# tszalay/poreseq

Hardware: AMD Instinct MI355X
Metric: kb consensus refined/sec at 10x coverage (higher is better)
Workload: dtype f64; 1 GPU; poreseq consensus, 10 kb region, 10x synthetic coverage (BASELINE configs[1]), full Mutate.py schedule per region; a step is 280 independent regions per GPU = 14 lock-step batches; the batches of the timed steps run step by step (a step's batches all finish before the next step's start) through 14 batch slots (host threads) per GPU; marshalling + H2D of the events, host greedy steps and D2H inside; region_bases=10000, events=10, regions_per_gpu=280, batches_in_flight=14, step_barrier=True, parallelism=280 regions x 1 GPU(s), 14 host thread(s) per GPU, no data-path collective

## Files before the change

poreseq_amd/csrc/ps_find.cpp:

```cpp
#include <algorithm>
#include <cmath>
#include <cstdlib>
#include <cstring>
#include <map>
#include <thread>

#include "ps_extract.h"
#include "ps_host.h"
#include "ps_sw.h"

namespace ps {

static bool likes_on_host() { const char* e = getenv("PORESEQ_DEBUG_LIKES_HOST"); return e && atoi(e) != 0; }

static void fillinds(SwResult& al) {
    if (al.a.empty()) return;
    int i1 = al.a[0], i2 = al.b[0];
    for (size_t k = 0; k < al.a.size(); k++) {
        if (al.a[k] > 0) i1 = al.a[k]; else al.a[k] = i1;
        if (al.b[k] > 0) i2 = al.b[k]; else al.b[k] = i2;
    }
}

namespace {
// ... 214 lines not shown
    for (size_t i = 1; i < st.size(); i++) {
        if (cur == st[i]) continue;
        bool hit = false;
        for (int n = 1; n <= 4 && !hit; n++)
            for (int k = 0; k < (1 << (2 * n)); k++)
                if (succ(cur, k, n) == st[i]) {
                    for (int b = 1; b <= n; b++) s.push_back(base_at(cur, b));
                    cur = st[i]; hit = true; break;
                }
        if (!hit) { cur = st[i]; s.push_back(base_at(cur, 0)); }
    }
    for (int b = 1; b <= 4; b++) s.push_back(base_at(cur, b));
    return s;
}

struct RandState {
    random_data rd;
    char st[128];
    bool init = false;
};
namespace { thread_local RandState t_rand; }
static void rs_seed(RandState* r, unsigned seed) {
    memset(&r->rd, 0, sizeof(r->rd));
    initstate_r(seed, r->st, sizeof(r->st), &r->rd);
    r->init = true;
}
static int rs_next(RandState* r) {
    if (!r->init) rs_seed(r, 1);
    int32_t v = 0;
    random_r(&r->rd, &v);
    return (int)v;
}
void rand_seed(unsigned seed) { rs_seed(&t_rand, seed); }
int rand_next() { return rs_next(&t_rand); }
RandState* rand_state_new(unsigned seed) { RandState* r = new RandState(); rs_seed(r, seed); return r; }
void rand_state_free(RandState* r) { delete r; }
void rand_state_seed(RandState* r, unsigned seed) { rs_seed(r, seed); }
int rand_state_next(RandState* r) { return rs_next(r ? r : &t_rand); }

namespace {
struct VitGather { std::vector<double> obsin; int T = 0; };
}

static int vit_refuses_refs(const Align& a, const char* who, int region) {
    for (int e = 0; e < a.E; e++) {
        const double* ra = a.h_ra.data() + a.off[e];
        for (int t = 0; t < a.n[e]; t++)
            if (ra[t] >= 2147483648.0) {
                char val[64];
                snprintf(val, sizeof(val), "%g", ra[t]);
                return fail(PS_ERR_BAD_ARG, std::string(who) + ": " + (region >= 0 ? "region " + std::to_string(region) + ": " : std::string()) + "event " + std::to_string(e) +
                                                ", level " + std::to_string(t) + ": ref_align = " + val + " is not below 2^31 (ViterbiMutate walks the positions from (int)ref_align)");
            }
    }
    return PS_OK;
}

static void vit_gather(const Align* a, const double* h_ri, const JobOut* info, VitGather* g) {
    const int E = a->E;
    int maxpos = 0;
    for (int e = 0; e < E; e++) {
        if (!info[e].has_index) continue;
        const double* ri = h_ri + a->off[e];
        for (int t = 0; t < a->n[e]; t++) {
            const double v = ri[t];
            if (v >= 0.0 && v < 1e9 && v == std::floor(v)) maxpos = std::max(maxpos, (int)v);
        }
    }
    std::vector<std::vector<int>> first(E);
    for (int e = 0; e < E; e++) {
        if (!info[e].has_index) continue;
        first[e].assign((size_t)maxpos + 2, -1);
        const double* ri = h_ri + a->off[e];
        for (int t = 0; t < a->n[e]; t++) {
            const double v = ri[t];
            if (v >= -1.0 && v <= (double)maxpos && v == std::floor(v)) {
                int& slot = first[e][(size_t)((int)v + 1)];
                if (slot < 0) slot = t;
            }
        }
    }
    auto rstart = [&](int e) { return info[e].has_index ? info[e].refstart : -1; };
    auto rend = [&](int e) { return info[e].has_index ? info[e].refend : -1; };
    int refind = rstart(0);
    for (int e = 0; e < E; e++) refind = std::min(refind, rstart(e));
    std::vector<double>& obsin = g->obsin;
    int T = 0;
    while (true) {
        int nl = 0, nal = 0;
        const size_t at = obsin.size();
        obsin.resize(at + (size_t)E * 4, 0.0);
        for (int e = 0; e < E; e++) {
            if (refind < -1 || refind > maxpos || first[e].empty() || first[e][refind + 1] < 0) continue;
            const double* ra = a->h_ra.data() + a->off[e];
            const double* mean = a->h_mean.data() + a->off[e];
            const double* stdv = a->h_stdv.data() + a->off[e];
            int t = first[e][refind + 1], cnt = 1;
            double lsum = 0, ssum = 0;
            lsum += mean[t]; ssum += stdv[t];
            for (t++; t < a->n[e] && ra[t] <= refind; t++)
                if (ra[t] > 0) { lsum += mean[t]; ssum += stdv[t]; cnt++; }
            const double lvl = lsum / cnt, sd = ssum / cnt;
            nl++;
            double* o = obsin.data() + at + (size_t)e * 4;
            o[0] = lvl; o[1] = sd; o[2] = std::log(sd); o[3] = 1.0;
        }
        for (int e = 0; e < E; e++) if (refind >= rstart(e) && refind <= rend(e)) nal++;
        if (nl <= nal * 0.2) {
            obsin.resize(at);
            if (nal == 0) break;
            refind++;
            continue;
        }
        T++;
        refind++;
    }
    g->T = T;
}

static void vit_draw(void* rng, double* rnd, size_t n) {
    RandState* r = (RandState*)rng;
    for (size_t k = 0; k < n; k++) rnd[k] = rand_state_next(r) / (double(RAND_MAX) + 1);
}

int viterbi_mutate_multi(Runtime* rt, const std::vector<Align*>& as, const std::vector<RandState*>& rngs, int nkeep, double skip, double stay,
                         double mmin, double mmax, const std::vector<std::vector<std::string>*>& outs, VitTap* tap, const char* who, bool lockstep) {
    Tick tk("viterbi_mutate");
    const int R = (int)as.size();
    for (int r = 0; r < R; r++) outs[r]->clear();
    std::vector<double*> h_ri(R, nullptr);
    std::vector<JobOut*> info(R, nullptr);
    for (int r = 0; r < R; r++) {
        PS_TRY(as[r]->refs_to_host_async(rt));
        as[r]->last_stream = (void*)rt->stream;
        PS_TRY(rt->down(&h_ri[r], as[r]->d_ri, (size_t)as[r]->ntot));
        PS_TRY(rt->down(&info[r], as[r]->d_out, (size_t)as[r]->E));
    }
    PS_HIP(hipStreamSynchronize(rt->stream));
    for (int r = 0; r < R; r++) as[r]->refs_finish();
    tk.lap("refs D2H");
    for (int r = 0; r < R; r++) PS_TRY(vit_refuses_refs(*as[r], who, lockstep ? r : -1));
    std::vector<VitGather> gath(R);
    par_for(R, [&](int r) { vit_gather(as[r], h_ri[r], info[r], &gath[r]); });
    tk.lap("gather levels");
    std::vector<VitRegionH> regs(R);
    for (int r = 0; r < R; r++) {
        regs[r].E = as[r]->E; regs[r].T = gath[r].T; regs[r].obsin = gath[r].obsin.data(); regs[r].d_model = as[r]->d_model;
        as[r]->last_stream = (void*)rt->stream;
        regs[r].rng = rngs[r]; regs[r].draw = vit_draw;
        regs[r].index = lockstep ? r : -1;
    }
    std::vector<std::vector<std::vector<int>>> paths;
    {
        auto need = [&](size_t k) { return 26.0 * 1024.0 * (double)regs[k].T + 32.0 * (double)regs[k].T * regs[k].E; };
        double cap = std::max(1e9, PLAN_VITERBI_FRAC * device_share_bytes());
        for (size_t k0 = 0; k0 < regs.size();) {
            size_t k1 = k0;
            double acc = 0;
            for (; k1 < regs.size(); k1++) { const double add = need(k1); if (k1 > k0 && acc + add > cap) break; acc += add; }
            std::vector<std::vector<std::vector<int>>> part;
            const int rc = viterbi_device_multi(rt, std::vector<VitRegionH>(regs.begin() + k0, regs.begin() + k1), nkeep, skip, stay, mmin, mmax, &part, tap, who);
            if (rc == PS_ERR_NOMEM && k1 - k0 > 1) { cap *= 0.5; continue; }
            PS_TRY(rc);
            for (auto& pr : part) paths.push_back(std::move(pr));
            k0 = k1;
        }
    }
    tk.lap("device");
    par_for(R, [&](int r) { for (auto& p : paths[r]) outs[r]->push_back(path_to_bases(p)); });
    tk.lap("paths to bases");
    return PS_OK;
}

int viterbi_mutate(Runtime* rt, Align* a, int nkeep, double skip, double stay, double mmin, double mmax,
                   std::vector<std::string>* out, bool verbose) {
    const int rc = viterbi_mutate_multi(rt, {a}, {nullptr}, nkeep, skip, stay, mmin, mmax, {out}, nullptr, "ps_viterbi_mutate", false);
    if (verbose && rc == PS_OK) {
        fputs("Viterbi", stderr);
        for (size_t k = 200; k <= a->bases.size(); k += 200) fputc('.', stderr);
        fputc('\n', stderr);
        fflush(stderr);
    }
    return rc;
}

}
```

poreseq_amd/csrc/ps_poison.h:

```cpp
#ifndef PS_POISON_H_
#define PS_POISON_H_

#include <cstring>

namespace ps {

enum class PoisonClass { INDEX = 0, VALUE = 1, EXEMPT = 2 };
struct PoisonEntry { const char* name; PoisonClass cls; const char* why; };

constexpr PoisonEntry POISON_TABLE[] = {
    {"jobs", PoisonClass::INDEX, "JobD: pointers, sizes, offsets"},
    {"states", PoisonClass::INDEX, "5-mer state ids and their -1 padding"},
    {"lb", PoisonClass::INDEX, "band centres per column"},
    {"lo", PoisonClass::INDEX, "lowest in-band row per anti-diagonal"},
    {"hi", PoisonClass::INDEX, "highest in-band row per anti-diagonal"},
    {"maxw", PoisonClass::INDEX, "widest footprint: sizes P"},
    {"fill_pairs", PoisonClass::INDEX, "job indices of paired fills"},
    {"rec", PoisonClass::INDEX, "records {main, stay} — and the Viterbi arena, whose back-pointer shorts the host follows as state ids (vit_follow_bp)"},
    {"flg", PoisonClass::INDEX, "step words and strip codes: the backtrace turns them into moves"},
    {"cmax", PoisonClass::VALUE, "per-column maxima of main: read by k_prefix and the edit kernels as max operands only"},
    {"pm", PoisonClass::VALUE, "prefix maxima over columns: compared and added, never indexed with"},
    {"best", PoisonClass::VALUE, "JobOut.best gathered per job: copied to the host and clamped at 0"},
    {"sw_jobs", PoisonClass::INDEX, "SweepJob: offsets and step counts"},
    {"sw_band", PoisonClass::INDEX, "row bounds per column"},
    {"sw_qlo", PoisonClass::INDEX, "lowest strip in band per step"},
    {"sw_qhi", PoisonClass::INDEX, "highest strip in band per step"},
    {"sw_sb", PoisonClass::INDEX, "StripBest: score with its cell"},
    {"sw_win", PoisonClass::INDEX, "widest window of strips: sizes the launch"},
    {"sw_pairs", PoisonClass::INDEX, "SwPair: lengths and offsets"},
    {"sw_chars", PoisonClass::INDEX, "sequence bytes, compared and used as substitution keys"},
    {"sw_row", PoisonClass::INDEX, "checkpoint rows of packed scores and directions"},
    {"sw_col", PoisonClass::INDEX, "checkpoint columns"},
    {"sw_blk", PoisonClass::INDEX, "block maxima with their cells"},
    {"sw_prog", PoisonClass::INDEX, "progress counters the blocks spin on"},
    {"sw_out", PoisonClass::INDEX, "index lists"},
    {"sw_res", PoisonClass::INDEX, "per-pair records: score, cell, list length"},
    {"sw_map_redo", PoisonClass::INDEX, "position tables of redone pairs"},
    {"seed_refs", PoisonClass::INDEX, "ref_align doubles are converted to column indices"},
    {"seed_out", PoisonClass::INDEX, "JobOut: cells and flags beside the score"},
    {"like_groups", PoisonClass::INDEX, "LikeGroup: job ranges and offsets"},
    {"like_out", PoisonClass::VALUE, "per-base likelihood sums: copied to the host and differenced"},
    {"remap_units", PoisonClass::INDEX, "unit descriptors of k_remap"},
    {"var_map", PoisonClass::INDEX, "position tables"},
    {"keep", PoisonClass::INDEX, "kept-column index per column"},
    {"mutint", PoisonClass::INDEX, "edit tables and descriptors"},
    {"mutdbl", PoisonClass::VALUE, "old / delta / score / oldall doubles: max and sum operands, copied to the host as scores"},
    {"ptable", PoisonClass::INDEX, "ps_point_best carries slots beside the scores"},
    {"support", PoisonClass::INDEX, "records with counts"},
    {"phase", PoisonClass::INDEX, "links, set ids, haplotype tags"},
    {"astats_in", PoisonClass::INDEX, "StatJob / StatRegion: pointers and sizes"},
    {"astats", PoisonClass::INDEX, "ps_event_stats and ps_kmer_cell carry counts"},
    {"vit_regs", PoisonClass::INDEX, "VitReg: pointers, sizes, offsets"},
    {"vit_posreg", PoisonClass::INDEX, "region of every position"},
    {"vit_in", PoisonClass::INDEX, "the fourth double of every record is the `present` flag"},
    {"vit_lik", PoisonClass::VALUE, "final scores per state: the host takes their argmax, a comparison of values"},
    {"vit_att", PoisonClass::INDEX, "default"},
    {"vit_start", PoisonClass::INDEX, "start state of the traces"},
    {"vit_rnd", PoisonClass::INDEX, "deviates: the picked state depends on them"},
    {"vit_path", PoisonClass::INDEX, "state paths"},
};

inline const PoisonEntry* poison_entry(const char* name) {
    for (const PoisonEntry& e : POISON_TABLE) if (!strcmp(e.name, name)) return &e;
    return nullptr;
}

}

#endif
```

poreseq_amd/csrc/ps_viterbi.hip:

```cpp
#include <atomic>

#include "ps_internal.h"
#include "ps_vitpath.h"

namespace ps {

struct ModelRowV { double mu, sg, lsg, sm, lam, llam; };
__device__ __forceinline__ double emission_v(const ModelRowV& m, double x, double sd, double lsd, double log2pi) {
    double d = (x - m.mu) / m.sg;
    double l = -0.5 * (d * d + log2pi) - m.lsg;
    double e = (sd - m.sm) / m.sm;
    l += 0.5 * (m.llam - 3 * lsd - log2pi - e * e * m.lam / sd);
    return l;
}

struct VitReg {
    const double* model;
    int E, T;
    int64_t in_off;
    int64_t t_off;
};

template <int VMAXE>
__global__ __launch_bounds__(256) void k_vit_obs(const VitReg* __restrict__ regs, const int* __restrict__ pos_reg, const double* __restrict__ obsin,
                                                 double log2pi, double* __restrict__ obs, double* __restrict__ eobs) {
    const int t = blockIdx.x;
    const VitReg R = regs[pos_reg[t]];
    const int E = R.E;
    const double* in = obsin + R.in_off + (size_t)(t - R.t_off) * E * 4;
    for (int st = threadIdx.x; st < NS; st += 256) {
        double v[VMAXE];
        int nl = 0;
        for (int e = 0; e < E; e++) {
            if (in[e * 4 + 3] == 0.0) continue;
            const double* gm = R.model + (size_t)e * 6 * NS;
            ModelRowV m = {gm[st], gm[NS + st], gm[2 * NS + st], gm[3 * NS + st], gm[4 * NS + st], gm[5 * NS + st]};
            const double l = emission_v(m, in[e * 4 + 0], in[e * 4 + 1], in[e * 4 + 2], log2pi);
            int k = nl++;
            while (k > 0 && v[k - 1] > l) { v[k] = v[k - 1]; k--; }
            v[k] = l;
        }
        double r;
        if (nl > 1) {
            int drop = (int)floor(nl * 0.25);
            if (drop > nl - 2) drop = 0;
            double s = 0.0;
            for (int k = drop; k < nl; k++) s += v[k];
            r = s / (double)(nl - drop);
        } else {
            r = nl == 1 ? v[0] : 0.0;
        }
        obs[(size_t)t * NS + st] = r;
        eobs[(size_t)t * NS + st] = exp(r);
    }
}

__global__ __launch_bounds__(256) void k_vit_obs_lds(const VitReg* __restrict__ regs, const int* __restrict__ pos_reg, const double* __restrict__ obsin,
                                                     double log2pi, double* __restrict__ obs, double* __restrict__ eobs) {
    extern __shared__ double vit_v[];
    const int t = blockIdx.x;
    const VitReg R = regs[pos_reg[t]];
    const int E = R.E;
    const double* in = obsin + R.in_off + (size_t)(t - R.t_off) * E * 4;
    double* v = vit_v + threadIdx.x;
    for (int st = threadIdx.x; st < NS; st += 256) {
        int nl = 0;
        for (int e = 0; e < E; e++) {
            if (in[e * 4 + 3] == 0.0) continue;
            const double* gm = R.model + (size_t)e * 6 * NS;
            ModelRowV m = {gm[st], gm[NS + st], gm[2 * NS + st], gm[3 * NS + st], gm[4 * NS + st], gm[5 * NS + st]};
            const double l = emission_v(m, in[e * 4 + 0], in[e * 4 + 1], in[e * 4 + 2], log2pi);
            int k = nl++;
            while (k > 0) {
                const double w = v[(k - 1) * 256];
                if (!(w > l)) break;
                v[k * 256] = w;
                k--;
            }
            v[k * 256] = l;
        }
        double r;
        if (nl > 1) {
            int drop = (int)floor(nl * 0.25);
            if (drop > nl - 2) drop = 0;
            double s = 0.0;
            for (int k = drop; k < nl; k++) s += v[k * 256];
            r = s / (double)(nl - drop);
        } else {
            r = nl == 1 ? v[0] : 0.0;
        }
        obs[(size_t)t * NS + st] = r;
        eobs[(size_t)t * NS + st] = exp(r);
    }
}

#define PS_LDS_BARRIER() asm volatile("s_waitcnt lgkmcnt(0)\n\ts_barrier" ::: "memory")

struct Fam { double mx, second, psum; int idx; int pad; };

__device__ __forceinline__ Fam fam_join(const Fam& A, const Fam& B) {
    Fam r;
    r.mx = fmax(A.mx, B.mx);
    const int ia = A.mx == r.mx ? A.idx : 0x7fffffff, ib = B.mx == r.mx ? B.idx : 0x7fffffff;
    r.idx = min(ia, ib);
    const double lower = A.mx == B.mx ? -BIG * 10 : fmin(A.mx, B.mx);
    r.second = fmax(fmax(A.second, B.second), lower);
    r.psum = A.psum + B.psum;
    r.pad = 0;
    return r;
}

template <int N>
__device__ __forceinline__ double row_shl(double v) {
    int lo = __double2loint(v), hi = __double2hiint(v);
    lo = __builtin_amdgcn_update_dpp(0, lo, 0x100 + N, 0xf, 0xf, true);
    hi = __builtin_amdgcn_update_dpp(0, hi, 0x100 + N, 0xf, 0xf, true);
    return __hiloint2double(hi, lo);
}
template <int N>
__device__ __forceinline__ Fam fam_shl(const Fam& f) {
    Fam o;
    o.mx = row_shl<N>(f.mx); o.second = row_shl<N>(f.second); o.psum = row_shl<N>(f.psum);
    o.idx = __builtin_amdgcn_update_dpp(0, f.idx, 0x100 + N, 0xf, 0xf, true); o.pad = 0;
    return o;
}
__device__ __forceinline__ double wave_sum(double v) {
    v += row_shl<1>(v); v += row_shl<2>(v); v += row_shl<4>(v); v += row_shl<8>(v);
    auto lane_d = [&](int l) {
        const int lo = __builtin_amdgcn_readlane(__double2loint(v), l), hi = __builtin_amdgcn_readlane(__double2hiint(v), l);
        return __hiloint2double(hi, lo);
    };
    return (lane_d(0) + lane_d(16)) + (lane_d(32) + lane_d(48));
}

__device__ __forceinline__ double below(double x) {
    long long b = __double_as_longlong(x);
    b += x < 0.0 ? 1 : -1;
    return __longlong_as_double(b);
}

#define VPAD(q) ((q) + ((q) >> 5))

__global__ __launch_bounds__(1024) void k_vit_steps(const VitReg* __restrict__ regs, const double* __restrict__ obs_all, const double* __restrict__ eobs_all,
                                                    double skip, double stay, double lskip, double lstay, double l25,
                                                    short* __restrict__ bp_all, double* __restrict__ lfwd_all,
                                                    double* __restrict__ lik_final_all, int keep_fwd) {
    const int T = regs[blockIdx.x].T;
    const size_t roff = (size_t)regs[blockIdx.x].t_off * NS;
    const double* __restrict__ obs = obs_all + roff;
    const double* __restrict__ eobs = eobs_all + roff;
    short* __restrict__ bp = bp_all + roff;
    double* __restrict__ lfwd_out = lfwd_all + (keep_fwd ? roff : 0);
    double* __restrict__ lik_final = lik_final_all + (size_t)blockIdx.x * NS;
    if (T <= 0) return;
    __shared__ double s_lik[2][NS + NS / 32], s_fwd[2][NS + NS / 32];
    __shared__ Fam s_fam[336];
    __shared__ double s_red[16];
    __shared__ double s_scale;
    const int c = threadIdx.x, lane = c & 63, wave = c >> 6;
    s_lik[0][VPAD(c)] = 0.0;
    s_fwd[0][VPAD(c)] = 1.0 / NS;
    if (c == 0) s_scale = 1.0;
    if (c < 16) s_red[c] = 1.0 / 16;
    __syncthreads();
    const double sp1 = 0.25, sp2 = sp1 * 0.25 * skip, sp3 = sp2 * 0.25 * skip;
    const double lsp1 = l25, lsp2 = lsp1 + l25 + lskip, lsp3 = lsp2 + l25 + lskip;
    int fj = 0, fg = 0, fq0 = 0, fqs = 0;
    if (c < 256) { fj = 1; fg = c; fq0 = c; fqs = 256; }
    else if (c < 512) { const int u = c - 256; fj = 2; fg = u >> 2; fq0 = fg + 256 * (u & 3); fqs = 64; }
    else if (c < 768) { const int u = c - 512; fj = 3; fg = u >> 4; fq0 = fg + 64 * (u & 15); fqs = 16; }
    int cur = 0;
    constexpr int VPF = 4;
    double oA[VPF], eA[VPF], oB[VPF], eB[VPF];
    const int TL = T - 1;
#define VIT_LOAD(O, E, t0)                                             \
    _Pragma("unroll") for (int u = 0; u < VPF; u++) {                   \
        const size_t at = (size_t)min((t0) + u, TL) * NS + c;           \
        O[u] = obs[at]; E[u] = eobs[at];                                \
    }
#define VIT_RUN(O, E, t0)                                               \
    _Pragma("unroll") for (int u = 0; u < VPF; u++) {                   \
        if ((t0) + u < T) vit_one((t0) + u, O[u], E[u]);                \
    }
    auto vit_one = [&](const int t, const double o, const double eo) {
        const double* pl = s_lik[cur];
        const double* pf = s_fwd[cur];
        if (fj) {
            Fam m[4];
#pragma unroll
            for (int k = 0; k < 4; k++) {
                const int q = fq0 + k * fqs;
                m[k].mx = pl[VPAD(q)]; m[k].idx = q; m[k].second = -BIG * 10; m[k].psum = pf[VPAD(q)]; m[k].pad = 0;
            }
            Fam f = fam_join(fam_join(m[0], m[1]), fam_join(m[2], m[3]));
            if (fj >= 2) { f = fam_join(f, fam_shl<1>(f)); f = fam_join(f, fam_shl<2>(f)); }
            if (fj == 3) { f = fam_join(f, fam_shl<4>(f)); f = fam_join(f, fam_shl<8>(f)); }
            const bool writer = fj == 1 || (fj == 2 && (c & 3) == 0) || (fj == 3 && (c & 15) == 0);
            if (writer) s_fam[(fj == 1 ? 0 : fj == 2 ? 256 : 320) + fg] = f;
        } else if (c == 1023) {
            double ptot = 0.0;
            for (int w = 0; w < 16; w++) ptot += s_red[w];
            int ex;
            frexp(ptot, &ex);
            s_scale = ldexp(1.0, min(-ex, 1000));
        }
        PS_LDS_BARRIER();
        double best = -BIG; int bq = -1; double fsum = 0.0;
#pragma unroll
        for (int j = 1; j <= 3; j++) {
            const int g = j == 1 ? (c >> 2) : j == 2 ? (c >> 4) : (c >> 6);
            const Fam f = s_fam[(j == 1 ? 0 : j == 2 ? 256 : 320) + g];
            const double a = o + (j == 1 ? lsp1 : j == 2 ? lsp2 : lsp3);
            const double m = a + f.mx;
            fsum += (j == 1 ? sp1 : j == 2 ? sp2 : sp3) * f.psum;
            if (f.second > -BIG * 5 && a + f.second == m) {
                const int cnt = 1 << (2 * j), sh = 10 - 2 * j;
                for (int k = 0; k < cnt; k++) {
                    const int q = g + (k << sh);
                    const double l = a + pl[VPAD(q)];
                    if (l > best) { best = l; bq = q; }
                }
            } else if (m > best) { best = m; bq = f.idx; }
        }
        {
            const double l = o + lstay + pl[VPAD(c)];
            if (l > best) { best = l; bq = c; }
            fsum += stay * pf[VPAD(c)];
        }
        const double nf = (fsum * s_scale) * eo;
        {
            const double wsum = wave_sum(nf);
            if (lane == 0) s_red[wave] = wsum;
        }
        s_lik[cur ^ 1][VPAD(c)] = best;
        s_fwd[cur ^ 1][VPAD(c)] = nf;
        bp[(size_t)t * NS + c] = (short)bq;
        if (keep_fwd) lfwd_out[(size_t)t * NS + c] = nf;
        PS_LDS_BARRIER();
        cur ^= 1;
    };
    VIT_LOAD(oA, eA, 0)
    for (int t0 = 0; t0 < T; t0 += 2 * VPF) {
        VIT_LOAD(oB, eB, t0 + VPF)
        VIT_RUN(oA, eA, t0)
        VIT_LOAD(oA, eA, t0 + 2 * VPF)
        VIT_RUN(oB, eB, t0 + VPF)
    }
#undef VIT_LOAD
#undef VIT_RUN
    lik_final[c] = s_lik[cur][VPAD(c)];
}

__device__ __forceinline__ double trans_weight(int cur, int p, double skip, double stay) {
    double t = 0.0, sp = 0.25;
#pragma unroll
    for (int j = 1; j <= 4; j++) {
        if ((p & ((1 << (10 - 2 * j)) - 1)) == (cur >> (2 * j))) t += sp;
        sp = sp * 0.25 * skip;
    }
    if (p == cur) t = stay;
    return t;
}

__global__ void k_vit_log(double* __restrict__ v, size_t n) {
    const size_t i = (size_t)blockIdx.x * blockDim.x + threadIdx.x;
    if (i < n) v[i] = log(v[i]);
}

template <int N>
__device__ __forceinline__ double row_shr(double v) {
    int lo = __double2loint(v), hi = __double2hiint(v);
    lo = __builtin_amdgcn_update_dpp(0, lo, 0x110 + N, 0xf, 0xf, true);
    hi = __builtin_amdgcn_update_dpp(0, hi, 0x110 + N, 0xf, 0xf, true);
    return __hiloint2double(hi, lo);
}
__device__ __forceinline__ double lane_get(double v, int l) {
    return __hiloint2double(__builtin_amdgcn_readlane(__double2hiint(v), l), __builtin_amdgcn_readlane(__double2loint(v), l));
}
__device__ __forceinline__ double wave_scan(double v, int lane) {
    v += row_shr<1>(v); v += row_shr<2>(v); v += row_shr<4>(v); v += row_shr<8>(v);
    const double t0 = lane_get(v, 15), t1 = lane_get(v, 31), t2 = lane_get(v, 47);
    const int row = lane >> 4;
    const double add = row == 0 ? 0.0 : row == 1 ? t0 : row == 2 ? t0 + t1 : (t0 + t1) + t2;
    return v + add;
}

constexpr int VT_THREADS = 512;
constexpr int VT_SPT = NS / VT_THREADS;
constexpr int VT_WAVES = VT_THREADS / 64;
__global__ __launch_bounds__(VT_THREADS) void k_vit_trace(const VitReg* __restrict__ regs, const double* __restrict__ lfwd_all, const int* __restrict__ starts,
                                                         double skip, double stay, const double* __restrict__ atten,
                                                         const double* __restrict__ rnd_all, short* __restrict__ path_all) {
    const int T = regs[blockIdx.y].T;
    if (T <= 0) return;
    const int start = starts[blockIdx.y];
    const double* __restrict__ lfwd = lfwd_all + (size_t)regs[blockIdx.y].t_off * NS;
    const double* __restrict__ rnd = rnd_all + (size_t)gridDim.x * regs[blockIdx.y].t_off;
    short* __restrict__ path = path_all + (size_t)gridDim.x * regs[blockIdx.y].t_off;
    __shared__ double s_wtot[2][VT_WAVES];
    __shared__ int s_pick[2][VT_WAVES];
    const int k = blockIdx.x, t = threadIdx.x, l = t & 63, w = t >> 6;
    const double at = atten[k];
    int cur = start;
    double2 lf = *(const double2*)(lfwd + (size_t)(T - 1) * NS + VT_SPT * t);
    double ex0 = exp(at * lf.x), ex1 = exp(at * lf.y);
    double rcur = rnd[(size_t)k * T];
    for (int i = T - 1; i >= 0; i--) {
        const int par = i & 1;
        if (t == 0) path[(size_t)k * T + i] = (short)cur;
        double2 nx = lf;
        double rnx = rcur;
        if (i > 0) { nx = *(const double2*)(lfwd + (size_t)(i - 1) * NS + VT_SPT * t); rnx = rnd[(size_t)k * T + (T - i)]; }
        const double tv0 = trans_weight(cur, VT_SPT * t, skip, stay), tv1 = trans_weight(cur, VT_SPT * t + 1, skip, stay);
        const double c0 = tv0 == 0.0 ? 0.0 : tv0 * ex0;
        const double c1 = c0 + (tv1 == 0.0 ? 0.0 : tv1 * ex1);
        const double nex0 = exp(at * nx.x), nex1 = exp(at * nx.y);
        const double incl = wave_scan(c1, l);
        if (l == 63) s_wtot[par][w] = incl;
        PS_LDS_BARRIER();
        double before = 0.0, total = 0.0;
#pragma unroll
        for (int q = 0; q < VT_WAVES; q++) {
            const double wq = s_wtot[par][q];
            if (q == w) before = total;
            total = q ? total + wq : wq;
        }
        const double base = before + (incl - c1);
        const double thr = rcur * total;
        int pick = 0x7fffffff;
        if (thr < base + c1) pick = thr < base + c0 ? VT_SPT * t : VT_SPT * t + 1;
        const unsigned long long hit = __builtin_amdgcn_ballot_w64(pick != 0x7fffffff);
        int wpick = 0x7fffffff;
        if (hit) wpick = __builtin_amdgcn_readlane(pick, __builtin_ctzll(hit));
        if (l == 0) s_pick[par][w] = wpick;
        PS_LDS_BARRIER();
        int pk = 0x7fffffff;
#pragma unroll
        for (int q = VT_WAVES - 1; q >= 0; q--) { const int pq = s_pick[par][q]; pk = pq != 0x7fffffff ? pq : pk; }
        cur = pk == 0x7fffffff ? NS - 1 : pk;
        lf = nx; rcur = rnx; ex0 = nex0; ex1 = nex1;
    }
}

int viterbi_device_multi(Runtime* rt, const std::vector<VitRegionH>& regions, int nkeep, double skip, double stay, double mmin, double mmax,
                         std::vector<std::vector<std::vector<int>>>* paths, VitTap* tap, const char* who) {
    const int R = (int)regions.size();
    paths->assign(R, {});
    std::vector<VitReg> regs(R);
    int64_t ttot = 0, intot = 0;
    int maxE = 0;
    for (int r = 0; r < R; r++) {
        regs[r].model = regions[r].d_model; regs[r].E = regions[r].E; regs[r].T = regions[r].T;
        regs[r].in_off = intot; regs[r].t_off = ttot;
        intot += (int64_t)regions[r].T * regions[r].E * 4; ttot += regions[r].T;
        maxE = std::max(maxE, regions[r].E);
    }
    if (tap)
        for (int r = 0; r < R; r++) { tap->T.push_back(regions[r].T); tap->paths.emplace_back(); tap->lik_final.insert(tap->lik_final.end(), NS, 0.0); }
    if (ttot <= 0) return PS_OK;
    if (maxE > 256) return fail(PS_ERR_UNSUPPORTED, "ViterbiMutate: more than 256 events");
    std::vector<int> pos_reg((size_t)ttot);
    for (int r = 0; r < R; r++) std::fill(pos_reg.begin() + regs[r].t_off, pos_reg.begin() + regs[r].t_off + regs[r].T, r);
    PS_TRY(rt->buf("vit_regs").ensure(R * sizeof(VitReg)));
    PS_TRY(rt->buf("vit_posreg").ensure((size_t)ttot * sizeof(int)));
    PS_TRY(rt->buf("vit_in").ensure((size_t)std::max<int64_t>(intot, 1) * sizeof(double)));
    auto al = [](size_t b) { return (b + 255) & ~(size_t)255; };
    const size_t b_obs = al((size_t)ttot * NS * sizeof(double)), b_fwd = al((size_t)(nkeep ? ttot : 1) * NS * sizeof(double)),
                 b_bp = al((size_t)ttot * NS * sizeof(short));
    DBuf& arena = rt->buf("rec");
    PS_TRY(arena.ensure(2 * b_obs + b_fwd + b_bp));
    PS_TRY(rt->buf("vit_lik").ensure((size_t)R * NS * sizeof(double)));
    if (nkeep > 0) {
        PS_TRY(rt->buf("vit_att").ensure(nkeep * sizeof(double)));
        PS_TRY(rt->buf("vit_start").ensure(R * sizeof(int)));
        PS_TRY(rt->buf("vit_rnd").ensure((size_t)nkeep * ttot * sizeof(double)));
        PS_TRY(rt->buf("vit_path").ensure((size_t)nkeep * ttot * sizeof(short)));
    }
    VitReg* d_regs = rt->buf("vit_regs").as<VitReg>();
    int* d_posreg = rt->buf("vit_posreg").as<int>();
    double* d_in = rt->buf("vit_in").as<double>();
    char* abase = (char*)arena.p;
    double* d_obs = (double*)abase;
    double* d_eobs = (double*)(abase + b_obs);
    double* d_fwd = (double*)(abase + 2 * b_obs);
    short* d_bp = (short*)(abase + 2 * b_obs + b_fwd);
    double* d_lik = rt->buf("vit_lik").as<double>();
    PS_TRY(rt->up(d_regs, regs.data(), R * sizeof(VitReg)));
    PS_TRY(rt->up(d_posreg, pos_reg.data(), (size_t)ttot * sizeof(int)));
    for (int r = 0; r < R; r++)
        if (regions[r].T && regions[r].E) PS_TRY(rt->up(d_in + regs[r].in_off, regions[r].obsin, (size_t)regions[r].T * regions[r].E * 4 * sizeof(double)));
    bool lds_ok = false;
    if (maxE <= 72) {
        static std::atomic<int> attr(0);
        if (attr.load(std::memory_order_acquire) == 0) {
            const hipError_t e = hipFuncSetAttribute((const void*)k_vit_obs_lds, hipFuncAttributeMaxDynamicSharedMemorySize, 160 * 1024);
            if (e != hipSuccess) (void)hipGetLastError();
            attr.store(e == hipSuccess ? 1 : -1, std::memory_order_release);
        }
        lds_ok = attr.load(std::memory_order_acquire) == 1;
    }
    int build = lds_ok ? 1 : maxE <= 64 ? 2 : 3;
    if (tap && tap->obs_build) {
        build = tap->obs_build;
        if (build < 1 || build > 3 || (build == 1 && !lds_ok) || (build == 2 && maxE > 64))
            return fail(PS_ERR_BAD_ARG, "ViterbiMutate: the emission build asked for does not take this many events");
    }
    prof_begin(rt);
    if (rt->prof_on && !(tap && tap->obs_rows)) rt->prof[build == 1 ? "vit_obs_lds" : (build == 2 ? "vit_obs_64" : "vit_obs_256")].launches++;
    if (tap && tap->obs_rows) {
        std::vector<double> eo((size_t)ttot * NS);
        for (size_t k = 0; k < eo.size(); k++) eo[k] = std::exp(tap->obs_rows[k]);
        PS_TRY(rt->up(d_obs, tap->obs_rows, eo.size() * sizeof(double)));
        PS_TRY(rt->up(d_eobs, eo.data(), eo.size() * sizeof(double)));
    } else if (build == 1)
        hipLaunchKernelGGL(k_vit_obs_lds, dim3((unsigned)ttot), dim3(256), (size_t)256 * std::max(maxE, 1) * sizeof(double), rt->stream, d_regs, d_posreg, d_in,
                           std::log(2 * M_PI), d_obs, d_eobs);
    else if (build == 2) hipLaunchKernelGGL(k_vit_obs<64>, dim3((unsigned)ttot), dim3(256), 0, rt->stream, d_regs, d_posreg, d_in, std::log(2 * M_PI), d_obs, d_eobs);
    else hipLaunchKernelGGL(k_vit_obs<256>, dim3((unsigned)ttot), dim3(256), 0, rt->stream, d_regs, d_posreg, d_in, std::log(2 * M_PI), d_obs, d_eobs);
    hipLaunchKernelGGL(k_vit_steps, dim3(R), dim3(1024), 0, rt->stream, d_regs, d_obs, d_eobs, skip, stay, std::log(skip), std::log(stay),
                       std::log(0.25), d_bp, d_fwd, d_lik, nkeep ? 1 : 0);
    PS_LAUNCH_CHECK();
    double* lik = nullptr;
    PS_TRY(rt->down(&lik, d_lik, (size_t)R * NS));
    double *tap_obs = nullptr, *tap_fwd = nullptr;
    short* tap_bp = nullptr;
    if (tap) {
        PS_TRY(rt->down(&tap_obs, d_obs, (size_t)ttot * NS));
        PS_TRY(rt->down(&tap_bp, d_bp, (size_t)ttot * NS));
        if (nkeep > 0) PS_TRY(rt->down(&tap_fwd, d_fwd, (size_t)ttot * NS));
    }
    double* h_rand = nullptr;
    if (nkeep > 0) {
        h_rand = (double*)rt->stage.alloc((size_t)nkeep * ttot * sizeof(double));
        if (!h_rand) return fail(PS_ERR_NOMEM, "hipHostMalloc (staging arena)");
        for (int r = 0; r < R; r++) regions[r].draw(regions[r].rng, h_rand + (size_t)nkeep * regs[r].t_off, (size_t)nkeep * regions[r].T);
    }
    PS_HIP(hipStreamSynchronize(rt->stream));
    if (tap) {
        tap->obs.insert(tap->obs.end(), tap_obs, tap_obs + (size_t)ttot * NS);
        tap->bp.insert(tap->bp.end(), tap_bp, tap_bp + (size_t)ttot * NS);
        if (tap_fwd) tap->fwd.insert(tap->fwd.end(), tap_fwd, tap_fwd + (size_t)ttot * NS);
        for (int r = 0; r < R; r++)
            if (regions[r].T) std::copy(lik + (size_t)r * NS, lik + (size_t)(r + 1) * NS, tap->lik_final.end() - (size_t)(R - r) * NS);
    }
    std::vector<int> starts(R, 0);
    for (int r = 0; r < R; r++) starts[r] = (int)(std::max_element(lik + (size_t)r * NS, lik + (size_t)(r + 1) * NS) - (lik + (size_t)r * NS));
    if (nkeep == 0) {
        short* bp = nullptr;
        PS_TRY(rt->down(&bp, d_bp, (size_t)ttot * NS));
        PS_HIP(hipStreamSynchronize(rt->stream));
        prof_end(rt, "viterbi", (double)ttot * NS * (8.0 * maxE + 8 + 2));
        for (int r = 0; r < R; r++) {
            if (!regions[r].T) continue;
            std::vector<int> p(regions[r].T);
            const int64_t dead = vit_follow_bp(bp, regs[r].t_off, regions[r].T, NS, starts[r], p.data());
            if (dead >= 0) {
                paths->assign(R, {});
                return fail(PS_ERR_BAD_ARG, std::string(who) + ": " + (regions[r].index >= 0 ? "region " + std::to_string(regions[r].index) + ": " : std::string()) +
                                                "no state is reachable at kept position " + std::to_string(dead) +
                                                " (every emission there is -inf or below -1e300, or the running scores have passed -1e300)");
            }
            (*paths)[r].push_back(p);
        }
        if (tap) std::copy(paths->begin(), paths->end(), tap->paths.end() - R);
        return PS_OK;
    }
    std::vector<double> att(nkeep);
    for (int k = 0; k < nkeep; k++) att[k] = mmin + (mmax - mmin) * k / (double)nkeep;
    PS_TRY(rt->up(rt->buf("vit_att").p, att.data(), nkeep * sizeof(double)));
    PS_TRY(rt->up(rt->buf("vit_start").p, starts.data(), R * sizeof(int)));
    PS_HIP(hipMemcpyAsync(rt->buf("vit_rnd").p, h_rand, (size_t)nkeep * ttot * sizeof(double), hipMemcpyHostToDevice, rt->stream));
    hipLaunchKernelGGL(k_vit_log, dim3((unsigned)(((size_t)ttot * NS + 255) / 256)), dim3(256), 0, rt->stream, d_fwd, (size_t)ttot * NS);
    hipLaunchKernelGGL(k_vit_trace, dim3(nkeep, R), dim3(VT_THREADS), 0, rt->stream, d_regs, d_fwd, rt->buf("vit_start").as<int>(), skip, stay,
                       rt->buf("vit_att").as<double>(), rt->buf("vit_rnd").as<double>(), rt->buf("vit_path").as<short>());
    PS_LAUNCH_CHECK();
    prof_end(rt, "viterbi", (double)ttot * NS * (8.0 * maxE + 8 + 2 + 8 + 8.0 * nkeep));
    short* hp = nullptr;
    PS_TRY(rt->down(&hp, rt->buf("vit_path").p, (size_t)nkeep * ttot));
    PS_HIP(hipStreamSynchronize(rt->stream));
    for (int r = 0; r < R; r++) {
        const int T = regions[r].T;
        if (!T) continue;
        const short* rp = hp + (size_t)nkeep * regs[r].t_off;
        for (int k = 0; k < nkeep; k++) {
            std::vector<int> p(T);
            for (int i = 0; i < T; i++) p[i] = rp[(size_t)k * T + i];
            (*paths)[r].push_back(p);
        }
    }
    if (tap) std::copy(paths->begin(), paths->end(), tap->paths.end() - R);
    return PS_OK;
}

}
```

poreseq_amd/csrc/ps_vitpath.h:

```cpp
#pragma once
#include <cstdint>

namespace ps {

inline int64_t vit_follow_bp(const int16_t* bp_all, int64_t t_off, int64_t T, int ns, int start, int* path) {
    int c = start;
    for (int64_t i = T - 1; i >= 0; i--) {
        path[i] = c;
        if (i == 0) break;
        const int q = bp_all[(t_off + i) * ns + c];
        if (q < 0) {
            int64_t j = i;
            for (; j > 0; j--) {
                const int16_t* row = bp_all + (t_off + j - 1) * ns;
                bool dead = true;
                for (int s = 0; s < ns && dead; s++) dead = row[s] < 0;
                if (!dead) break;
            }
            return j;
        }
        c = q;
    }
    return -1;
}

}
```

Baseline: 223.8 kb/s.

## Chunk Viterbi emission build over positions and drop the eobs table

The LDS emission kernel now handles up to 8 positions per block, so each model row loaded from global memory is reused across several positions. Blocks are described by chunk descriptors instead of a per-position region table. The exp(obs) table is no longer stored; k_vit_steps computes exp on the fly unless a tap supplies rows. The separate log kernel is folded into the forward step, which writes log(nf) directly. These changes cut memory traffic, one launch and arena size, at the cost of extra exp per step and more LDS per block, which may lower occupancy.

```diff
diff --git a/poreseq_amd/csrc/ps_find.cpp b/poreseq_amd/csrc/ps_find.cpp
--- a/poreseq_amd/csrc/ps_find.cpp
+++ b/poreseq_amd/csrc/ps_find.cpp
@@ -390,7 +390,8 @@
     }
     std::vector<std::vector<std::vector<int>>> paths;
     {
-        auto need = [&](size_t k) { return 26.0 * 1024.0 * (double)regs[k].T + 32.0 * (double)regs[k].T * regs[k].E; };
+        const double per_pos = (tap ? 26.0 : 18.0) * 1024.0;
+        auto need = [&](size_t k) { return per_pos * (double)regs[k].T + 32.0 * (double)regs[k].T * regs[k].E; };
         double cap = std::max(1e9, PLAN_VITERBI_FRAC * device_share_bytes());
         for (size_t k0 = 0; k0 < regs.size();) {
             size_t k1 = k0;
diff --git a/poreseq_amd/csrc/ps_poison.h b/poreseq_amd/csrc/ps_poison.h
--- a/poreseq_amd/csrc/ps_poison.h
+++ b/poreseq_amd/csrc/ps_poison.h
@@ -51,7 +51,7 @@
     {"astats_in", PoisonClass::INDEX, "StatJob / StatRegion: pointers and sizes"},
     {"astats", PoisonClass::INDEX, "ps_event_stats and ps_kmer_cell carry counts"},
     {"vit_regs", PoisonClass::INDEX, "VitReg: pointers, sizes, offsets"},
-    {"vit_posreg", PoisonClass::INDEX, "region of every position"},
+    {"vit_chunks", PoisonClass::INDEX, "VitChunk: region, first position, count"},
     {"vit_in", PoisonClass::INDEX, "the fourth double of every record is the `present` flag"},
     {"vit_lik", PoisonClass::VALUE, "final scores per state: the host takes their argmax, a comparison of values"},
     {"vit_att", PoisonClass::INDEX, "default"},
diff --git a/poreseq_amd/csrc/ps_viterbi.hip b/poreseq_amd/csrc/ps_viterbi.hip
--- a/poreseq_amd/csrc/ps_viterbi.hip
+++ b/poreseq_amd/csrc/ps_viterbi.hip
@@ -22,10 +22,10 @@
 };
 
 template <int VMAXE>
-__global__ __launch_bounds__(256) void k_vit_obs(const VitReg* __restrict__ regs, const int* __restrict__ pos_reg, const double* __restrict__ obsin,
-                                                 double log2pi, double* __restrict__ obs, double* __restrict__ eobs) {
-    const int t = blockIdx.x;
-    const VitReg R = regs[pos_reg[t]];
+__global__ __launch_bounds__(256) void k_vit_obs(const VitReg* __restrict__ regs, const VitChunk* __restrict__ chunks, const double* __restrict__ obsin,
+                                                 double log2pi, double* __restrict__ obs) {
+    const int t = chunks[blockIdx.x].first;
+    const VitReg R = regs[chunks[blockIdx.x].region];
     const int E = R.E;
     const double* in = obsin + R.in_off + (size_t)(t - R.t_off) * E * 4;
     for (int st = threadIdx.x; st < NS; st += 256) {
@@ -51,46 +51,64 @@
             r = nl == 1 ? v[0] : 0.0;
         }
         obs[(size_t)t * NS + st] = r;
-        eobs[(size_t)t * NS + st] = exp(r);
-    }
-}
-
-__global__ __launch_bounds__(256) void k_vit_obs_lds(const VitReg* __restrict__ regs, const int* __restrict__ pos_reg, const double* __restrict__ obsin,
-                                                     double log2pi, double* __restrict__ obs, double* __restrict__ eobs) {
+    }
+}
+
+template <int P>
+__global__ __launch_bounds__(256) void k_vit_obs_chunk(const VitReg* __restrict__ regs, const VitChunk* __restrict__ chunks, const double* __restrict__ obsin,
+                                                       int VE, double log2pi, double* __restrict__ obs) {
     extern __shared__ double vit_v[];
-    const int t = blockIdx.x;
-    const VitReg R = regs[pos_reg[t]];
-    const int E = R.E;
-    const double* in = obsin + R.in_off + (size_t)(t - R.t_off) * E * 4;
+    const VitChunk C = chunks[blockIdx.x];
+    const VitReg R = regs[C.region];
+    const int E = R.E, n = min(C.count, P);
+    const size_t in_pos = (size_t)E * 4, lst = (size_t)VE * 256;
+    const double* in = obsin + R.in_off + (size_t)(C.first - R.t_off) * in_pos;
     double* v = vit_v + threadIdx.x;
     for (int st = threadIdx.x; st < NS; st += 256) {
-        int nl = 0;
+        int nl[P];
+#pragma unroll
+        for (int p = 0; p < P; p++) nl[p] = 0;
         for (int e = 0; e < E; e++) {
-            if (in[e * 4 + 3] == 0.0) continue;
+            bool any = false;
+#pragma unroll
+            for (int p = 0; p < P; p++) any = any || (p < n && in[p * in_pos + e * 4 + 3] != 0.0);
+            if (!any) continue;
             const double* gm = R.model + (size_t)e * 6 * NS;
-            ModelRowV m = {gm[st], gm[NS + st], gm[2 * NS + st], gm[3 * NS + st], gm[4 * NS + st], gm[5 * NS + st]};
-            const double l = emission_v(m, in[e * 4 + 0], in[e * 4 + 1], in[e * 4 + 2], log2pi);
-            int k = nl++;
-            while (k > 0) {
-                const double w = v[(k - 1) * 256];
-                if (!(w > l)) break;
-                v[k * 256] = w;
-                k--;
+            const ModelRowV m = {gm[st], gm[NS + st], gm[2 * NS + st], gm[3 * NS + st], gm[4 * NS + st], gm[5 * NS + st]};
+#pragma unroll
+            for (int p = 0; p < P; p++) {
+                if (p >= n) continue;
+                const double* ip = in + p * in_pos + e * 4;
+                if (ip[3] == 0.0) continue;
+                const double l = emission_v(m, ip[0], ip[1], ip[2], log2pi);
+                double* vp = v + p * lst;
+                int k = nl[p]++;
+                while (k > 0) {
+                    const double w = vp[(k - 1) * 256];
+                    if (!(w > l)) break;
+                    vp[k * 256] = w;
+                    k--;
+                }
+                vp[k * 256] = l;
             }
-            v[k * 256] = l;
-        }
-        double r;
-        if (nl > 1) {
-            int drop = (int)floor(nl * 0.25);
-            if (drop > nl - 2) drop = 0;
-            double s = 0.0;
-            for (int k = drop; k < nl; k++) s += v[k * 256];
-            r = s / (double)(nl - drop);
-        } else {
-            r = nl == 1 ? v[0] : 0.0;
-        }
-        obs[(size_t)t * NS + st] = r;
-        eobs[(size_t)t * NS + st] = exp(r);
+        }
+#pragma unroll
+        for (int p = 0; p < P; p++) {
+            if (p >= n) continue;
+            const double* vp = v + p * lst;
+            const int np = nl[p];
+            double r;
+            if (np > 1) {
+                int drop = (int)floor(np * 0.25);
+                if (drop > np - 2) drop = 0;
+                double s = 0.0;
+                for (int k = drop; k < np; k++) s += vp[k * 256];
+                r = s / (double)(np - drop);
+            } else {
+                r = np == 1 ? vp[0] : 0.0;
+            }
+            obs[(size_t)(C.first + p) * NS + st] = r;
+        }
     }
 }
 
@@ -141,16 +159,18 @@
 
 #define VPAD(q) ((q) + ((q) >> 5))
 
+template <bool TABLE>
 __global__ __launch_bounds__(1024) void k_vit_steps(const VitReg* __restrict__ regs, const double* __restrict__ obs_all, const double* __restrict__ eobs_all,
                                                     double skip, double stay, double lskip, double lstay, double l25,
-                                                    short* __restrict__ bp_all, double* __restrict__ lfwd_all,
+                                                    short* __restrict__ bp_all, double* __restrict__ lfwd_all, double* __restrict__ raw_all,
                                                     double* __restrict__ lik_final_all, int keep_fwd) {
     const int T = regs[blockIdx.x].T;
     const size_t roff = (size_t)regs[blockIdx.x].t_off * NS;
     const double* __restrict__ obs = obs_all + roff;
-    const double* __restrict__ eobs = eobs_all + roff;
+    const double* __restrict__ eobs = TABLE ? eobs_all + roff : nullptr;
     short* __restrict__ bp = bp_all + roff;
     double* __restrict__ lfwd_out = lfwd_all + (keep_fwd ? roff : 0);
+    double* __restrict__ raw_out = raw_all ? raw_all + roff : nullptr;
     double* __restrict__ lik_final = lik_final_all + (size_t)blockIdx.x * NS;
     if (T <= 0) return;
     __shared__ double s_lik[2][NS + NS / 32], s_fwd[2][NS + NS / 32];
@@ -176,11 +196,12 @@
 #define VIT_LOAD(O, E, t0)                                             \
     _Pragma("unroll") for (int u = 0; u < VPF; u++) {                   \
         const size_t at = (size_t)min((t0) + u, TL) * NS + c;           \
-        O[u] = obs[at]; E[u] = eobs[at];                                \
+        O[u] = obs[at];                                                 \
+        if (TABLE) E[u] = eobs[at];                                     \
     }
 #define VIT_RUN(O, E, t0)                                               \
     _Pragma("unroll") for (int u = 0; u < VPF; u++) {                   \
-        if ((t0) + u < T) vit_one((t0) + u, O[u], E[u]);                \
+        if ((t0) + u < T) vit_one((t0) + u, O[u], TABLE ? E[u] : exp(O[u])); \
     }
     auto vit_one = [&](const int t, const double o, const double eo) {
         const double* pl = s_lik[cur];
@@ -235,7 +256,10 @@
         s_lik[cur ^ 1][VPAD(c)] = best;
         s_fwd[cur ^ 1][VPAD(c)] = nf;
         bp[(size_t)t * NS + c] = (short)bq;
-        if (keep_fwd) lfwd_out[(size_t)t * NS + c] = nf;
+        if (keep_fwd) {
+            lfwd_out[(size_t)t * NS + c] = log(nf);
+            if (raw_out) raw_out[(size_t)t * NS + c] = nf;
+        }
         PS_LDS_BARRIER();
         cur ^= 1;
     };
@@ -260,11 +284,6 @@
     }
     if (p == cur) t = stay;
     return t;
-}
-
-__global__ void k_vit_log(double* __restrict__ v, size_t n) {
-    const size_t i = (size_t)blockIdx.x * blockDim.x + threadIdx.x;
-    if (i < n) v[i] = log(v[i]);
 }
 
 template <int N>
@@ -359,16 +378,40 @@
         for (int r = 0; r < R; r++) { tap->T.push_back(regions[r].T); tap->paths.emplace_back(); tap->lik_final.insert(tap->lik_final.end(), NS, 0.0); }
     if (ttot <= 0) return PS_OK;
     if (maxE > 256) return fail(PS_ERR_UNSUPPORTED, "ViterbiMutate: more than 256 events");
-    std::vector<int> pos_reg((size_t)ttot);
-    for (int r = 0; r < R; r++) std::fill(pos_reg.begin() + regs[r].t_off, pos_reg.begin() + regs[r].t_off + regs[r].T, r);
+    constexpr size_t LDS_GRANT = 160 * 1024, LDS_BUDGET = 96 * 1024;
+    bool lds_ok = false;
+    if (maxE <= 72) {
+        static std::atomic<int> attr(0);
+        if (attr.load(std::memory_order_acquire) == 0) {
+            bool all = true;
+            for (const void* f : {(const void*)k_vit_obs_chunk<1>, (const void*)k_vit_obs_chunk<2>, (const void*)k_vit_obs_chunk<4>, (const void*)k_vit_obs_chunk<8>}) {
+                const hipError_t e = hipFuncSetAttribute(f, hipFuncAttributeMaxDynamicSharedMemorySize, (int)LDS_GRANT);
+                if (e != hipSuccess) { (void)hipGetLastError(); all = false; }
+            }
+            attr.store(all ? 1 : -1, std::memory_order_release);
+        }
+        lds_ok = attr.load(std::memory_order_acquire) == 1;
+    }
+    int build = lds_ok ? 1 : maxE <= 64 ? 2 : 3;
+    if (tap && tap->obs_build) {
+        build = tap->obs_build;
+        if (build < 1 || build > 3 || (build == 1 && !lds_ok) || (build == 2 && maxE > 64))
+            return fail(PS_ERR_BAD_ARG, "ViterbiMutate: the emission build asked for does not take this many events");
+    }
+    const char* env_p = getenv("PORESEQ_DEBUG_VIT_CHUNK");
+    const int P = build == 1 ? vit_chunk_positions(maxE, LDS_BUDGET, LDS_GRANT, env_p ? std::max(atoi(env_p), 0) : 0) : 1;
+    std::vector<int> Ts(R);
+    for (int r = 0; r < R; r++) Ts[r] = regions[r].T;
+    const std::vector<VitChunk> chunks = vit_chunks(Ts, P);
     PS_TRY(rt->buf("vit_regs").ensure(R * sizeof(VitReg)));
-    PS_TRY(rt->buf("vit_posreg").ensure((size_t)ttot * sizeof(int)));
+    PS_TRY(rt->buf("vit_chunks").ensure(chunks.size() * sizeof(VitChunk)));
     PS_TRY(rt->buf("vit_in").ensure((size_t)std::max<int64_t>(intot, 1) * sizeof(double)));
     auto al = [](size_t b) { return (b + 255) & ~(size_t)255; };
     const size_t b_obs = al((size_t)ttot * NS * sizeof(double)), b_fwd = al((size_t)(nkeep ? ttot : 1) * NS * sizeof(double)),
                  b_bp = al((size_t)ttot * NS * sizeof(short));
+    const size_t b_raw = tap && nkeep ? b_obs : 0, b_eobs = tap && tap->obs_rows ? b_obs : 0;
     DBuf& arena = rt->buf("rec");
-    PS_TRY(arena.ensure(2 * b_obs + b_fwd + b_bp));
+    PS_TRY(arena.ensure(b_obs + b_fwd + b_bp + b_raw + b_eobs));
     PS_TRY(rt->buf("vit_lik").ensure((size_t)R * NS * sizeof(double)));
     if (nkeep > 0) {
         PS_TRY(rt->buf("vit_att").ensure(nkeep * sizeof(double)));
@@ -377,48 +420,41 @@
         PS_TRY(rt->buf("vit_path").ensure((size_t)nkeep * ttot * sizeof(short)));
     }
     VitReg* d_regs = rt->buf("vit_regs").as<VitReg>();
-    int* d_posreg = rt->buf("vit_posreg").as<int>();
+    VitChunk* d_chunks = rt->buf("vit_chunks").as<VitChunk>();
     double* d_in = rt->buf("vit_in").as<double>();
     char* abase = (char*)arena.p;
     double* d_obs = (double*)abase;
-    double* d_eobs = (double*)(abase + b_obs);
-    double* d_fwd = (double*)(abase + 2 * b_obs);
-    short* d_bp = (short*)(abase + 2 * b_obs + b_fwd);
+    double* d_fwd = (double*)(abase + b_obs);
+    short* d_bp = (short*)(abase + b_obs + b_fwd);
+    double* d_raw = b_raw ? (double*)(abase + b_obs + b_fwd + b_bp) : nullptr;
+    double* d_eobs = b_eobs ? (double*)(abase + b_obs + b_fwd + b_bp + b_raw) : nullptr;
     double* d_lik = rt->buf("vit_lik").as<double>();
     PS_TRY(rt->up(d_regs, regs.data(), R * sizeof(VitReg)));
-    PS_TRY(rt->up(d_posreg, pos_reg.data(), (size_t)ttot * sizeof(int)));
+    PS_TRY(rt->up(d_chunks, chunks.data(), chunks.size() * sizeof(VitChunk)));
     for (int r = 0; r < R; r++)
         if (regions[r].T && regions[r].E) PS_TRY(rt->up(d_in + regs[r].in_off, regions[r].obsin, (size_t)regions[r].T * regions[r].E * 4 * sizeof(double)));
-    bool lds_ok = false;
-    if (maxE <= 72) {
-        static std::atomic<int> attr(0);
-        if (attr.load(std::memory_order_acquire) == 0) {
-            const hipError_t e = hipFuncSetAttribute((const void*)k_vit_obs_lds, hipFuncAttributeMaxDynamicSharedMemorySize, 160 * 1024);
-            if (e != hipSuccess) (void)hipGetLastError();
-            attr.store(e == hipSuccess ? 1 : -1, std::memory_order_release);
-        }
-        lds_ok = attr.load(std::memory_order_acquire) == 1;
-    }
-    int build = lds_ok ? 1 : maxE <= 64 ? 2 : 3;
-    if (tap && tap->obs_build) {
-        build = tap->obs_build;
-        if (build < 1 || build > 3 || (build == 1 && !lds_ok) || (build == 2 && maxE > 64))
-            return fail(PS_ERR_BAD_ARG, "ViterbiMutate: the emission build asked for does not take this many events");
-    }
     prof_begin(rt);
     if (rt->prof_on && !(tap && tap->obs_rows)) rt->prof[build == 1 ? "vit_obs_lds" : (build == 2 ? "vit_obs_64" : "vit_obs_256")].launches++;
+    const double log2pi = std::log(2 * M_PI);
+    const dim3 ogrid((unsigned)chunks.size());
     if (tap && tap->obs_rows) {
         std::vector<double> eo((size_t)ttot * NS);
         for (size_t k = 0; k < eo.size(); k++) eo[k] = std::exp(tap->obs_rows[k]);
         PS_TRY(rt->up(d_obs, tap->obs_rows, eo.size() * sizeof(double)));
         PS_TRY(rt->up(d_eobs, eo.data(), eo.size() * sizeof(double)));
-    } else if (build == 1)
-        hipLaunchKernelGGL(k_vit_obs_lds, dim3((unsigned)ttot), dim3(256), (size_t)256 * std::max(maxE, 1) * sizeof(double), rt->stream, d_regs, d_posreg, d_in,
-                           std::log(2 * M_PI), d_obs, d_eobs);
-    else if (build == 2) hipLaunchKernelGGL(k_vit_obs<64>, dim3((unsigned)ttot), dim3(256), 0, rt->stream, d_regs, d_posreg, d_in, std::log(2 * M_PI), d_obs, d_eobs);
-    else hipLaunchKernelGGL(k_vit_obs<256>, dim3((unsigned)ttot), dim3(256), 0, rt->stream, d_regs, d_posreg, d_in, std::log(2 * M_PI), d_obs, d_eobs);
-    hipLaunchKernelGGL(k_vit_steps, dim3(R), dim3(1024), 0, rt->stream, d_regs, d_obs, d_eobs, skip, stay, std::log(skip), std::log(stay),
-                       std::log(0.25), d_bp, d_fwd, d_lik, nkeep ? 1 : 0);
+    } else if (build == 1) {
+        const int VE = std::max(maxE, 1);
+        const size_t lds = (size_t)P * VE * 256 * sizeof(double);
+        auto kern = P == 1 ? k_vit_obs_chunk<1> : P == 2 ? k_vit_obs_chunk<2> : P <= 4 ? k_vit_obs_chunk<4> : k_vit_obs_chunk<8>;
+        hipLaunchKernelGGL(kern, ogrid, dim3(256), lds, rt->stream, d_regs, d_chunks, d_in, VE, log2pi, d_obs);
+    } else if (build == 2) hipLaunchKernelGGL(k_vit_obs<64>, ogrid, dim3(256), 0, rt->stream, d_regs, d_chunks, d_in, log2pi, d_obs);
+    else hipLaunchKernelGGL(k_vit_obs<256>, ogrid, dim3(256), 0, rt->stream, d_regs, d_chunks, d_in, log2pi, d_obs);
+    if (d_eobs)
+        hipLaunchKernelGGL(k_vit_steps<true>, dim3(R), dim3(1024), 0, rt->stream, d_regs, d_obs, d_eobs, skip, stay, std::log(skip), std::log(stay),
+                           std::log(0.25), d_bp, d_fwd, d_raw, d_lik, nkeep ? 1 : 0);
+    else
+        hipLaunchKernelGGL(k_vit_steps<false>, dim3(R), dim3(1024), 0, rt->stream, d_regs, d_obs, (const double*)nullptr, skip, stay, std::log(skip), std::log(stay),
+                           std::log(0.25), d_bp, d_fwd, d_raw, d_lik, nkeep ? 1 : 0);
     PS_LAUNCH_CHECK();
     double* lik = nullptr;
     PS_TRY(rt->down(&lik, d_lik, (size_t)R * NS));
@@ -427,7 +463,7 @@
     if (tap) {
         PS_TRY(rt->down(&tap_obs, d_obs, (size_t)ttot * NS));
         PS_TRY(rt->down(&tap_bp, d_bp, (size_t)ttot * NS));
-        if (nkeep > 0) PS_TRY(rt->down(&tap_fwd, d_fwd, (size_t)ttot * NS));
+        if (nkeep > 0) PS_TRY(rt->down(&tap_fwd, d_raw, (size_t)ttot * NS));
     }
     double* h_rand = nullptr;
     if (nkeep > 0) {
@@ -470,7 +506,6 @@
     PS_TRY(rt->up(rt->buf("vit_att").p, att.data(), nkeep * sizeof(double)));
     PS_TRY(rt->up(rt->buf("vit_start").p, starts.data(), R * sizeof(int)));
     PS_HIP(hipMemcpyAsync(rt->buf("vit_rnd").p, h_rand, (size_t)nkeep * ttot * sizeof(double), hipMemcpyHostToDevice, rt->stream));
-    hipLaunchKernelGGL(k_vit_log, dim3((unsigned)(((size_t)ttot * NS + 255) / 256)), dim3(256), 0, rt->stream, d_fwd, (size_t)ttot * NS);
     hipLaunchKernelGGL(k_vit_trace, dim3(nkeep, R), dim3(VT_THREADS), 0, rt->stream, d_regs, d_fwd, rt->buf("vit_start").as<int>(), skip, stay,
                        rt->buf("vit_att").as<double>(), rt->buf("vit_rnd").as<double>(), rt->buf("vit_path").as<short>());
     PS_LAUNCH_CHECK();
diff --git a/poreseq_amd/csrc/ps_vitpath.h b/poreseq_amd/csrc/ps_vitpath.h
--- a/poreseq_amd/csrc/ps_vitpath.h
+++ b/poreseq_amd/csrc/ps_vitpath.h
@@ -1,5 +1,8 @@
 #pragma once
+#include <algorithm>
+#include <cstddef>
 #include <cstdint>
+#include <vector>
 
 namespace ps {
 
@@ -24,4 +27,25 @@
     return -1;
 }
 
+struct VitChunk { int32_t region, first, count; };
+
+inline std::vector<VitChunk> vit_chunks(const std::vector<int>& T, int P) {
+    std::vector<VitChunk> out;
+    P = std::max(P, 1);
+    int64_t t_off = 0;
+    for (size_t r = 0; r < T.size(); r++) {
+        for (int64_t t = 0; t < T[r]; t += P) out.push_back({(int32_t)r, (int32_t)(t_off + t), (int32_t)std::min<int64_t>(P, T[r] - t)});
+        t_off += std::max(T[r], 0);
+    }
+    return out;
 }
+
+constexpr int VIT_CHUNK_MAX = 8;
+inline int vit_chunk_positions(int VE, size_t budget, size_t grant, int forced) {
+    const size_t one = (size_t)std::max(VE, 1) * 256 * sizeof(double);
+    const size_t room = forced > 0 ? grant : std::min(budget, grant);
+    const int fit = (int)std::min<size_t>(room / one, VIT_CHUNK_MAX);
+    return std::max(1, forced > 0 ? std::min(forced, fit) : fit);
+}
+
+}
```

Result: slower. 214.9 kb/s (-4.0%).
